# AbrahamSanders/realtime-codec-agent

Hardware: AMD Instinct MI355X
Metric: batch-encode audio-hours/hour (+ xRT and p50 frame-step latency of 1 duplex stream in `duplex`) (higher is better)
Workload: dtype f32; 1 GPU; batch MagiCodec-style encode, 16 kHz stereo, 0.1 s chunks / 2.0 s context, 256 windows per step (BASELINE configs[1]); codebook=131072x16

## Files before the change

include/rca.h:

```cpp
#ifndef RCA_H
#define RCA_H

#include <stdint.h>

#ifdef __cplusplus
extern "C" {
#endif

#define RCA_OK 0
#define RCA_ERR_ARG -1
#define RCA_ERR_HIP -2
#define RCA_ERR_STATE -3
#define RCA_ERR_MISSING -4

#define RCA_MAX_STAGES 8

typedef struct rca_codec rca_codec_t;
typedef struct rca_lm rca_lm_t;

#define RCA_F32 0
#define RCA_BF16 1
#define RCA_Q8_0 2
#define RCA_F16 3
#define RCA_Q6_K 5
// ... 57 lines not shown
typedef struct {
    int64_t src_off;
    int64_t n_in;
    int64_t dst_off;
    int32_t src_stride;
    int32_t n_mix;
} rca_ingest_row_t;
int rca_codec_ingest_rows_dev(rca_codec_t* h, const void* src_dev, int64_t src_span, int32_t src_fmt, const rca_ingest_row_t* rows_dev,
                              const rca_ingest_row_t* rows_host, int32_t n_rows, int32_t up, int32_t down, const float* taps_host,
                              int32_t n_taps, float* dst_dev, int64_t dst_span, void* stream);
int rca_codec_ingest_supported(const rca_codec_t* h, int32_t up, int32_t down, int32_t n_taps);

int rca_codec_encode_tail_dev(rca_codec_t* h, const float* pcm_dev, int32_t B, int32_t T, int32_t n_keep,
                              int64_t* codes_dev, void* stream);
int rca_codec_decode_tail_dev(rca_codec_t* h, const int64_t* codes_dev, int32_t B, int32_t F, int32_t n_samples,
                              float* pcm_dev, void* stream);
int rca_codec_decode_rows_dev(rca_codec_t* h, const int64_t* codes_dev, const int64_t* src_off_dev, int32_t B, int32_t F, int32_t n_samples,
                              float* pcm_dev, const int64_t* dst_off_dev, int64_t code_span, int64_t pcm_span, void* stream);
int rca_codec_decode_error(rca_codec_t* h, void* stream, int32_t* raised);

#define RCA_JOIN_HEAD 1
#define RCA_JOIN_TAIL 2
typedef struct {
    int64_t seg_off;
    int64_t n;
    int64_t out_off;
    int32_t flags;
    int32_t reserved;
} rca_join_seg_t;
int rca_codec_crossfade_join_dev(rca_codec_t* h, const float* seg_dev, int64_t seg_span, const rca_join_seg_t* segs_dev,
                                 const rca_join_seg_t* segs_host, int32_t n_segs, const float* fade_in_dev, int32_t n_fade, float* out_dev,
                                 int64_t out_span, void* stream);

int rca_codec_encode_tail(rca_codec_t* h, const float* pcm_host, int32_t B, int32_t T, int32_t n_keep, int64_t* codes_host);
int rca_codec_decode_tail(rca_codec_t* h, const int64_t* codes_host, int32_t B, int32_t F, int32_t n_samples, float* pcm_host);
int rca_codec_set_stream_graphs(rca_codec_t* h, int32_t enable);
int rca_codec_set_mfma_mode(rca_codec_t* h, int32_t mode);
int rca_codec_receptive_field(const rca_codec_t* h, int32_t* enc_left_frames, int32_t* dec_left_frames);
int rca_codec_set_window_trim(rca_codec_t* h, int32_t enable);

int rca_codec_decode(rca_codec_t* h, const int64_t* codes_host, int32_t B, int32_t F, float* pcm_host);
int rca_codec_decode_dev(rca_codec_t* h, const int64_t* codes_dev, int32_t B, int32_t F, float* pcm_dev,
                         void* stream);

int rca_codec_encoder_dev(rca_codec_t* h, const float* pcm_dev, int32_t B, int32_t T, float* ze_dev, void* stream);
int rca_codec_quantize_dev(rca_codec_t* h, const float* ze_dev, int64_t rows, int64_t* codes_dev, void* stream);
int rca_codec_decoder_dev(rca_codec_t* h, const float* zq_dev, int32_t B, int32_t F, float* pcm_dev, void* stream);
int rca_codec_codebook_dev(rca_codec_t* h, const float** out_dev);

int rca_codec_codebook(rca_codec_t* h, float* out_host);

int rca_codec_encode_tap(rca_codec_t* h, const float* pcm_host, int32_t B, int32_t T, int32_t layer,
                         float* out_host, int64_t out_numel);

int rca_codec_encode_tap_bf16(rca_codec_t* h, const float* pcm_host, int32_t B, int32_t T, int32_t layer,
                              uint16_t* hi_host, uint16_t* lo_host, int64_t numel);

#define RCA_KCLASS_CHAIN 1
#define RCA_KCLASS_MFMA_32x32 2
#define RCA_KCLASS_MFMA_64x32 3
#define RCA_KCLASS_MFMA_32x64 4
#define RCA_KCLASS_MFMA_64x64 5
#define RCA_KCLASS_WS 6
#define RCA_KCLASS_BF16 7
#define RCA_KCLASS_MFMA_OTHER 8
#define RCA_KCLASS_LDS 16
int rca_codec_decoder_layer_tap(rca_codec_t* h, int32_t layer, int32_t route, const float* x_host, int32_t B, int32_t Lin,
                                float* y_host, int64_t y_numel, int32_t* kernel_class, int32_t* guards_ok);

int rca_codec_set_variant(rca_codec_t* h, int32_t variant);

int rca_codec_profile(rca_codec_t* h, int32_t enable);
int rca_codec_profile_read(rca_codec_t* h, int32_t kclass, double* total_ms, int64_t* launches, double* flops,
                           double* bytes);

typedef struct {
    int32_t vocab_size;
    int32_t hidden;
    int32_t n_layers;
    int32_t n_heads;
    int32_t n_kv_heads;
    int32_t head_dim;
    int32_t ffn;
    int32_t n_ctx;
    float rms_eps;
    float rope_theta;
    int32_t rope_scaling;
    float rope_factor;
    float rope_low_freq_factor;
    float rope_high_freq_factor;
    int32_t rope_orig_ctx;
    int32_t logits_all;
    int32_t decode_weights;
} rca_lm_config_t;

typedef struct {
    int32_t top_k;
    float top_p;
    float min_p;
    float temp;
    uint32_t seed;
    int32_t n_bias;
    const int32_t* bias_ids;
    const float* bias_vals;
    float repeat_penalty;
    float freq_penalty;
// ... 135 lines not shown
```

realtime_codec_agent_amd/_native.py:

```python
from __future__ import annotations

import ctypes as C
import os
import subprocess
from typing import Dict, Iterable, List, Optional, Tuple

import numpy as np

_PKG_DIR = os.path.dirname(os.path.abspath(__file__))
CSRC_DIR = os.path.join(_PKG_DIR, "csrc")
LIB_PATH = os.environ.get("RCA_LIB_PATH") or os.path.join(_PKG_DIR, "librca_hip.so")
HIP_SOURCES = ["rca_codec.hip", "rca_lm.hip"]
HIPCC_FLAGS = ["--offload-arch=gfx950", "-O3", "-ffp-contract=off", "-std=c++17", "-fPIC", "-shared",
               "-Wno-unused-result", "-mllvm", "-amdgpu-kernarg-preload-count=14"]

MAX_STAGES = 8
RCA_F32, RCA_BF16, RCA_Q8_0, RCA_F16, RCA_Q4_K, RCA_Q6_K, RCA_Q5_K, RCA_Q4_0, RCA_Q4_1, RCA_IQ4_NL, RCA_IQ4_XS = 0, 1, 2, 3, 4, 5, 6, 7, 8, 9, 10


class RcaError(RuntimeError):
    pass


class Q8Blocks:
# ... 355 lines not shown
    import fcntl
    obj_dir = os.path.join(CSRC_DIR, ".obj")
    os.makedirs(obj_dir, exist_ok=True)
    with open(os.path.join(obj_dir, ".lock"), "w") as lock:
        fcntl.flock(lock, fcntl.LOCK_EX)
        if not force and not needs_build():
            return LIB_PATH
        headers = [os.path.join(CSRC_DIR, f) for f in os.listdir(CSRC_DIR) if f.endswith(".h")]
        headers.append(os.path.join(os.path.dirname(_PKG_DIR), "include", "rca.h"))
        hdr_t = max([os.path.getmtime(p) for p in headers if os.path.exists(p)] + [0.0])
        sfx = f".{os.getpid()}.tmp"
        objs, jobs = [], []
        for src in sources():
            obj = os.path.join(obj_dir, f"{os.path.splitext(os.path.basename(src))[0]}.{key}.o")
            objs.append(obj)
            if force or not os.path.exists(obj) or os.path.getmtime(obj) < max(os.path.getmtime(src), hdr_t):
                cmd = [hipcc] + cflags + ["-c", src, "-o", obj + sfx]
                if verbose:
                    print(" ".join(cmd))
                jobs.append((subprocess.Popen(cmd), cmd, obj))
        tmps = [obj + sfx for _, _, obj in jobs] + [LIB_PATH + sfx]
        try:
            failed = [cmd for p, cmd, _ in jobs if p.wait() != 0]
            if failed:
                raise subprocess.CalledProcessError(1, failed[0])
            for _, _, obj in jobs:
                os.replace(obj + sfx, obj)
            cmd = [hipcc, "--offload-arch=gfx950", "-shared", "-fPIC"] + objs + ["-o", LIB_PATH + sfx]
            if verbose:
                print(" ".join(cmd))
            subprocess.check_call(cmd)
            os.replace(LIB_PATH + sfx, LIB_PATH)
            with open(_stamp_path() + sfx, "w") as f:
                f.write(key + "\n")
            os.replace(_stamp_path() + sfx, _stamp_path())
        finally:
            for t in tmps + [_stamp_path() + sfx]:
                if os.path.exists(t):
                    os.remove(t)
    return LIB_PATH


_lib = None

ABI_SYMBOLS = [
    "rca_last_error", "rca_device_count", "rca_device_sync", "rca_version",
    "rca_codec_create", "rca_codec_destroy", "rca_codec_hop", "rca_codec_num_frames",
    "rca_codec_encode", "rca_codec_encode_dev", "rca_codec_encode_windows_dev", "rca_codec_encode_chunk_range_dev", "rca_codec_encode_rows_dev",
    "rca_codec_ingest_rows_dev", "rca_codec_ingest_supported",
    "rca_codec_decode_rows_dev", "rca_codec_decode_error", "rca_codec_crossfade_join_dev",
    "rca_codec_decode", "rca_codec_decode_dev",
    "rca_codec_encode_tail_dev", "rca_codec_decode_tail_dev", "rca_codec_encode_tail", "rca_codec_decode_tail", "rca_codec_set_stream_graphs", "rca_codec_receptive_field", "rca_codec_set_window_trim",
    "rca_codec_encoder_dev", "rca_codec_quantize_dev", "rca_codec_decoder_dev", "rca_codec_codebook_dev",
    "rca_codec_codebook", "rca_codec_encode_tap", "rca_codec_encode_tap_bf16", "rca_codec_set_variant", "rca_codec_sync",
    "rca_codec_profile", "rca_codec_profile_read",
    "rca_lm_create", "rca_lm_create_random", "rca_lm_destroy", "rca_lm_reset", "rca_lm_eval",
    "rca_lm_get_n_tokens", "rca_lm_set_n_tokens", "rca_lm_get_logits", "rca_lm_get_logits_row",
    "rca_lm_logits_dev", "rca_lm_sampler_init", "rca_lm_sample", "rca_lm_step", "rca_lm_token_probs",
    "rca_lm_sync", "rca_lm_set_graphs", "rca_lm_mask_head_rows", "rca_lm_set_mfma_prefill", "rca_lm_set_logits_all",
    "rca_lm_persist_codec_embeddings", "rca_lm_create_shared", "rca_lm_eval_async", "rca_lm_copy_kv", "rca_lm_swap_kv",
    "rca_lm_set_low_priority", "rca_lm_frame", "rca_lm_weight_format", "rca_lm_set_attn_fuse", "rca_lm_prefill_route",
    "rca_lm_set_act_format", "rca_lm_get_act_format", "rca_lm_gemv_tap", "rca_lm_kv_remove", "rca_lm_kv_read",
    "rca_lm_kv_write", "rca_lm_attn_tap", "rca_lm_score", "rca_lm_score_rows_tap", "rca_lm_put_logits",
    "rca_lm_set_kv_format", "rca_lm_get_kv_format", "rca_lm_kv_bytes_per_position", "rca_lm_kv_read_q8",
    "rca_duplex_frame", "rca_codec_workspace_sig", "rca_codec_stream_handoff", "rca_codec_codebook_size", "rca_codec_set_mfma_mode", "rca_lm_step_probe", "rca_duplex_prepare", "rca_duplex_precapture",
    "rca_lm_group_create", "rca_lm_group_destroy", "rca_lm_group_step",
    "rca_lm_batch_create", "rca_lm_batch_destroy", "rca_lm_batch_step", "rca_lm_batch_frame",
    "rca_lm_batch_frame_sel", "rca_lm_batch_captures", "rca_duplex_batch_frame", "rca_lm_batch_step_sel",
    "rca_lm_batch_eval", "rca_lm_kv_remove_many", "rca_lm_kv_remove_many_staged",
    "rca_codec_decoder_layer_tap", "rca_quantize_rows",
]


def lib():
    global _lib
    if _lib is not None:
        return _lib
    if not os.path.exists(LIB_PATH):
        raise RcaError(
            f"{LIB_PATH} not found: build the HIP extension first (python -c 'import __graft_entry__ as g; g.build()'). "
            "There is no CPU fallback for the product path."
        )
    import torch
    try:
        _lib = C.CDLL(LIB_PATH)
    except OSError as e:
        raise RcaError(f"cannot load {LIB_PATH}: {e}") from e
    _lib.rca_last_error.restype = C.c_char_p
    _lib.rca_version.restype = C.c_char_p
    _lib.rca_lm_batch_step_sel.argtypes = BATCH_STEP_SEL_ARGTYPES
    _lib.rca_lm_batch_step_sel.restype = C.c_int
    if hasattr(_lib, "rca_lm_batch_eval"):
        _lib.rca_lm_batch_eval.argtypes = BATCH_EVAL_ARGTYPES
        _lib.rca_lm_batch_eval.restype = C.c_int
    if hasattr(_lib, "rca_codec_decoder_layer_tap"):
        _lib.rca_codec_decoder_layer_tap.argtypes = DECODER_LAYER_TAP_ARGTYPES
        _lib.rca_codec_decoder_layer_tap.restype = C.c_int
    if hasattr(_lib, "rca_quantize_rows"):
        _lib.rca_quantize_rows.argtypes = QUANTIZE_ROWS_ARGTYPES
        _lib.rca_quantize_rows.restype = C.c_int
    for name in ("rca_lm_kv_remove_many", "rca_lm_kv_remove_many_staged"):
        if hasattr(_lib, name):
            getattr(_lib, name).argtypes = KV_REMOVE_MANY_ARGTYPES
            getattr(_lib, name).restype = C.c_int
    return _lib


# ... 44 lines not shown
```

realtime_codec_agent_amd/codec.py:

```python
from __future__ import annotations

import ctypes as C
from typing import Dict, Optional, Tuple

import numpy as np

from . import _native as N
from .codec_model import CodecConfig, init_codec_weights


class HipCodec:
    def __init__(self, cfg: CodecConfig, weights: Dict[str, np.ndarray], device: int = 0):
        self.cfg = cfg
        self.device = device
        self._lib = N.lib()
        self._h = C.c_void_p()
        tensors, keep = N.make_tensors(weights)
        ccfg = N.codec_config_c(cfg)
        N.check(self._lib.rca_codec_create(C.byref(ccfg), tensors, len(weights), device, C.byref(self._h)), "rca_codec_create")
        del keep
        self.hop = cfg.hop
        self.mfma_mode = 0

    def close(self):
# ... 37 lines not shown
    def encode_tail(self, pcm: np.ndarray, n_keep: int) -> np.ndarray:
        pcm = np.ascontiguousarray(pcm, dtype=np.float32)
        if pcm.ndim != 2:
            raise ValueError("pcm must be [B,T]")
        B, T = pcm.shape
        n_keep = min(int(n_keep), self.num_frames(T))
        codes = np.empty((B, n_keep), np.int64)
        N.check(self._lib.rca_codec_encode_tail(self._h, C.c_void_p(pcm.ctypes.data), B, T, n_keep, C.c_void_p(codes.ctypes.data)),
                "rca_codec_encode_tail")
        return codes

    def decode_tail(self, codes: np.ndarray, n_samples: int) -> np.ndarray:
        codes = np.ascontiguousarray(codes, dtype=np.int64)
        if codes.ndim != 2:
            raise ValueError("codes must be [B,F]")
        B, F = codes.shape
        n = min(int(n_samples), F * self.hop)
        pcm = np.empty((B, n), np.float32)
        N.check(self._lib.rca_codec_decode_tail(self._h, C.c_void_p(codes.ctypes.data), B, F, n, C.c_void_p(pcm.ctypes.data)),
                "rca_codec_decode_tail")
        return pcm

    def set_mfma_mode(self, mode: int) -> None:
        N.check(self._lib.rca_codec_set_mfma_mode(self._h, int(mode)), "rca_codec_set_mfma_mode")
        self.mfma_mode = int(mode)

    def set_stream_graphs(self, enable: bool) -> None:
        N.check(self._lib.rca_codec_set_stream_graphs(self._h, int(bool(enable))), "rca_codec_set_stream_graphs")

    def codebook(self) -> np.ndarray:
        out = np.empty((self.cfg.codebook_size, self.cfg.codebook_dim), np.float32)
        N.check(self._lib.rca_codec_codebook(self._h, C.c_void_p(out.ctypes.data)), "rca_codec_codebook")
        return out

    def encode_tap(self, pcm: np.ndarray, layer: int) -> np.ndarray:
        pcm = np.ascontiguousarray(pcm, dtype=np.float32)
        B, T = pcm.shape
        F = self.num_frames(T)
        n = self.cfg.n_stages
        L = F * self.hop
        if layer == 0:
            shape = (B, self.cfg.channels[0], L)
        elif layer <= n:
            for i in range(layer):
                L //= self.cfg.strides[i]
            shape = (B, self.cfg.channels[layer], L)
        elif layer == n + 1:
            shape = (B, self.cfg.latent_dim, F)
        else:
            shape = (B * F, self.cfg.codebook_dim)
        out = np.empty(shape, np.float32)
        N.check(self._lib.rca_codec_encode_tap(self._h, C.c_void_p(pcm.ctypes.data), B, T, layer, C.c_void_p(out.ctypes.data),
                                               C.c_int64(out.size)), "rca_codec_encode_tap")
        return out

    def encode_tap_bf16(self, pcm: np.ndarray, layer: int) -> Tuple[np.ndarray, Optional[np.ndarray]]:
        pcm = np.ascontiguousarray(pcm, dtype=np.float32)
        B, T = pcm.shape
        L = self.num_frames(T) * self.hop
        for i in range(layer):
            L //= self.cfg.strides[i]
        Cn = self.cfg.channels[layer] if 0 <= layer <= self.cfg.n_stages else 0
        hi = np.empty((B, Cn // 16, L, 16), np.uint16)
        lo = np.empty_like(hi) if self.mfma_mode == 3 else None
        N.check(self._lib.rca_codec_encode_tap_bf16(self._h, C.c_void_p(pcm.ctypes.data), B, T, layer, C.c_void_p(hi.ctypes.data),
                                                    C.c_void_p(lo.ctypes.data if lo is not None else None), C.c_int64(B * Cn * L)),
                "rca_codec_encode_tap_bf16")
        unblock = lambda a: np.ascontiguousarray(a.transpose(0, 1, 3, 2).reshape(B, Cn, L))
        return unblock(hi), (unblock(lo) if lo is not None else None)

    def decoder_layer_tap(self, layer: int, route: int, x: np.ndarray) -> Tuple[np.ndarray, int, bool]:
        x = np.ascontiguousarray(x, dtype=np.float32)
        layers = self.cfg.decoder_layers()
        if x.ndim != 3 or not 0 <= layer < len(layers) or x.shape[1] != layers[layer]["cin"]:
            raise ValueError("x must be [B, Cin, Lin] of a decoder layer")
        ly = layers[layer]
        B, _, Lin = x.shape
        y = np.empty((B, ly["cout"], Lin * ly["s"] if ly["tr"] else Lin), np.float32)
        kclass, guards = C.c_int32(-1), C.c_int32(-1)
        fp = C.POINTER(C.c_float)
        N.check(self._lib.rca_codec_decoder_layer_tap(self._h, layer, route, x.ctypes.data_as(fp), B, Lin, y.ctypes.data_as(fp),
                                                      C.c_int64(y.size), C.byref(kclass), C.byref(guards)), "rca_codec_decoder_layer_tap")
        return y, kclass.value, bool(guards.value)

    def encode_dev(self, pcm_ptr: int, B: int, T: int, codes_ptr: int, stream: int = 0) -> None:
        N.check(self._lib.rca_codec_encode_dev(self._h, C.c_void_p(pcm_ptr), B, T, C.c_void_p(codes_ptr), C.c_void_p(stream)), "rca_codec_encode_dev")

    def decode_dev(self, codes_ptr: int, B: int, F: int, pcm_ptr: int, stream: int = 0) -> None:
        N.check(self._lib.rca_codec_decode_dev(self._h, C.c_void_p(codes_ptr), B, F, C.c_void_p(pcm_ptr), C.c_void_p(stream)), "rca_codec_decode_dev")

    def encode_tail_dev(self, pcm_ptr: int, B: int, T: int, n_keep: int, codes_ptr: int, stream: int = 0) -> None:
        N.check(self._lib.rca_codec_encode_tail_dev(self._h, C.c_void_p(pcm_ptr), B, T, n_keep, C.c_void_p(codes_ptr), C.c_void_p(stream)),
                "rca_codec_encode_tail_dev")

    def decode_tail_dev(self, codes_ptr: int, B: int, F: int, n_samples: int, pcm_ptr: int, stream: int = 0) -> None:
        N.check(self._lib.rca_codec_decode_tail_dev(self._h, C.c_void_p(codes_ptr), B, F, n_samples, C.c_void_p(pcm_ptr), C.c_void_p(stream)),
                "rca_codec_decode_tail_dev")

    def receptive_field(self) -> Tuple[int, int]:
        a, b = C.c_int32(), C.c_int32()
        N.check(self._lib.rca_codec_receptive_field(self._h, C.byref(a), C.byref(b)), "rca_codec_receptive_field")
        return a.value, b.value

    def set_window_trim(self, enable: bool) -> None:
        N.check(self._lib.rca_codec_set_window_trim(self._h, int(bool(enable))), "rca_codec_set_window_trim")

# ... 280 lines not shown
```

realtime_codec_agent_amd/csrc/rca_codec.hip:

```cpp
#include <stdarg.h>

#include <algorithm>
#include <array>
#include <cmath>
#include <map>
#include <type_traits>

#include "rca_common.h"
#include "rca_conv_balance.h"

namespace rca {
thread_local char g_err[512] = {0};
}
using namespace rca;

typedef float f32x16 __attribute__((ext_vector_type(16)));

#define RCA_LAT_MAX_FRAMES 64
#define RCA_LDS_BUDGET (152 * 1024)

typedef float f32x4 __attribute__((ext_vector_type(4)));

struct RowSrc {
    const float* base;
// ... 1508 lines not shown
    for (int ft = 0; ft < FN; ++ft) {
        const long f = f0 + ft * 32 + (lane & 31);
#pragma unroll
        for (int kp = 0; kp < 8; ++kp) zb[ft][kp] = f < F ? z[f * 16 + 2 * kp + half] : 0.0f;
    }
    float best[FN];
    unsigned bidx[FN];
#pragma unroll
    for (int ft = 0; ft < FN; ++ft) { best[ft] = -INFINITY; bidx[ft] = 0xFFFFFFFFu; }

    for (int tile = tile_beg + wave; tile < tile_end; tile += 4) {
        const float4* ap = reinterpret_cast<const float4*>(cbp) + ((long)tile * 2) * 64 + lane;
        const float4 a0 = ap[0], a1 = ap[64];
        const float av[8] = {a0.x, a0.y, a0.z, a0.w, a1.x, a1.y, a1.z, a1.w};
        const int c0 = tile * 32;
        f32x16 cinit;
#pragma unroll
        for (int g = 0; g < 4; ++g) {
            const float4 h4 = *reinterpret_cast<const float4*>(hc + c0 + 8 * g + 4 * half);
            cinit[4 * g + 0] = h4.x; cinit[4 * g + 1] = h4.y; cinit[4 * g + 2] = h4.z; cinit[4 * g + 3] = h4.w;
        }
#pragma unroll
        for (int ft = 0; ft < FN; ++ft) {
            f32x16 acc = cinit;
#pragma unroll
            for (int kp = 0; kp < 8; ++kp) acc = __builtin_amdgcn_mfma_f32_32x32x2f32(av[kp], zb[ft][kp], acc, 0, 0, 0);
#pragma unroll
            for (int r = 0; r < 16; ++r) {
                const unsigned c = (unsigned)(c0 + (r & 3) + 8 * (r >> 2) + 4 * half);
                if (acc[r] > best[ft]) { best[ft] = acc[r]; bidx[ft] = c; }
            }
        }
    }
    __shared__ unsigned long long red[FN][4][32];
#pragma unroll
    for (int ft = 0; ft < FN; ++ft) {
        unsigned long long key = bidx[ft] == 0xFFFFFFFFu ? 0ull : pack_key(best[ft], bidx[ft]);
        const unsigned long long other = __shfl_xor(key, 32);
        key = other > key ? other : key;
        if (lane < 32) red[ft][wave][lane] = key;
    }
    __syncthreads();
    for (int i = threadIdx.x; i < FN * 32; i += 256) {
        const int ft = i >> 5, l = i & 31;
        const long f = f0 + i;
        if (f < F) {
            unsigned long long key = red[ft][0][l];
            for (int w = 1; w < 4; ++w) key = red[ft][w][l] > key ? red[ft][w][l] : key;
            atomicMax(&keys[f], key);
        }
    }
}

struct RowDst {
    int64_t* base;
    int C;
    long chan_stride;
    long win_stride;
    int fc;
    const long* row_off = nullptr;
};
__global__ __launch_bounds__(256) void vq_finalize_kernel(unsigned long long* __restrict__ keys, RowDst dst, long rows) {
    const long i = (long)blockIdx.x * blockDim.x + threadIdx.x;
    if (i >= rows) return;
    const unsigned long long key = keys[i];
    keys[i] = 0ull;
    const long b = i / dst.fc;
    const int j = (int)(i - b * dst.fc);
    dst.base[(dst.row_off ? dst.row_off[b] : (b % dst.C) * dst.chan_stride + (b / dst.C) * dst.win_stride) + j] =
        key == 0ull ? (int64_t)0 : (int64_t)(0xFFFFFFFFu - (unsigned)(key & 0xFFFFFFFFull));
}

__global__ __launch_bounds__(256) void embed_codes_kernel(const int64_t* __restrict__ codes, long ldc, const float* __restrict__ cb,
                                                          float* __restrict__ zq, int B, int F, int J, int N,
                                                          int* __restrict__ err) {
    const long idx = (long)blockIdx.x * blockDim.x + threadIdx.x;
    if (idx >= (long)B * J * F) return;
    const int f = (int)(idx % F);
    const long r = idx / F;
    const int j = (int)(r % J);
    const int b = (int)(r / J);
    int64_t c = codes[(long)b * ldc + f];
    if (c < 0 || c >= N) { atomicExch(err, 1); c = 0; }
    zq[idx] = cb[c * J + j];
}

__global__ __launch_bounds__(256) void embed_rows_kernel(const int64_t* __restrict__ codes, const long* __restrict__ src_off, int f0, int Frow,
                                                         long span, const float* __restrict__ cb, float* __restrict__ zq, int B, int F, int J,
                                                         int N, int* __restrict__ err) {
    const long idx = (long)blockIdx.x * blockDim.x + threadIdx.x;
    if (idx >= (long)B * J * F) return;
    const int f = (int)(idx % F);
    const long r = idx / F;
    const int j = (int)(r % J);
    const int b = (int)(r / J);
    const long o = src_off[b];
    int64_t c = -1;
    if (o >= 0 && o <= span - Frow) c = codes[o + f0 + f];
    if (c < 0 || c >= N) { atomicExch(err, 1); c = 0; }
    zq[idx] = cb[c * J + j];
}

__global__ __launch_bounds__(256) void scatter_tail_kernel(const float* __restrict__ src, long T, int n, float* __restrict__ dst,
                                                           const long* __restrict__ dst_off, long span, int B, int* __restrict__ err) {
    const long idx = (long)blockIdx.x * blockDim.x + threadIdx.x;
    if (idx >= (long)B * n) return;
// ... 1215 lines not shown
        const float slope = c.leaky_slope;
        const int Lout = L / E1.s;
        {
            ProfScope ps(h, st, 0, 2.0 * E1.cin * E1.k * E1.cout * (double)B * Lout + 2.0 * E0.k * E0.cout * (double)B * L,
                         4.0 * ((double)B * src.T + (double)B * E1.cout * Lout + (double)E1.cin * E1.k * E1.cout));
            prev_post = handoff(2, Lout);
            const int act = (E1.pre ? 1 : 0) | (prev_post ? 2 : 0);
            if (h->variant == 2 && try_conv_ws(E1, nullptr, y, B, L, Lout, slope, st, &fin)) { rc = RCA_OK; RCA_LAUNCH_CHECK(); }
            else if (E1.k == 4) rc = launch_conv_mfma<4, 2, 4>(E1, nullptr, y, B, L, Lout, slope, st, &fin, act, h->mfma_mode);
            else if (E1.k == 8) rc = launch_conv_mfma<8, 4, RCA_CIC_K8>(E1, nullptr, y, B, L, Lout, slope, st, &fin, act, h->mfma_mode);
            else rc = launch_conv_mfma<16, 8, RCA_CIC_K16>(E1, nullptr, y, B, L, Lout, slope, st, &fin, act, h->mfma_mode);
        }
        if (rc != RCA_OK) return rc;
        L = Lout;
        first = 2;
        if (tap_layer == 1) RCA_HIP(hipMemcpyAsync(tap_dev, y, (size_t)B * E1.cout * L * 4, hipMemcpyDeviceToDevice, st));
    } else if (h->lat_mode && !src.row_off && src.win_stride == 0 && src.C == B &&
               try_conv_lds(h, h->enc[0], src.base, src.chan_stride, src.T, h->act[cur].as<float>(), B, L, 0, st)) {
        RCA_LAUNCH_CHECK();
    } else {
        const ConvLayer& L0 = h->enc[0];
        const long total = (long)B * L;
        float* y = h->act[cur].as<float>();
        ProfScope ps(h, st, 2, 2.0 * L0.k * L0.cout * (double)total, 4.0 * ((double)total + (double)total * L0.cout));
        if (L0.k == 7) conv_in_kernel<7><<<cdiv(total, 256), 256, 0, st>>>(src, L0.w, L0.b, y, B, L0.cout, L);
        else if (L0.k == 5) conv_in_kernel<5><<<cdiv(total, 256), 256, 0, st>>>(src, L0.w, L0.b, y, B, L0.cout, L);
        else conv_in_kernel<3><<<cdiv(total, 256), 256, 0, st>>>(src, L0.w, L0.b, y, B, L0.cout, L);
        RCA_LAUNCH_CHECK();
        if (tap_layer == 0) RCA_HIP(hipMemcpyAsync(tap_dev, y, (size_t)B * L0.cout * L * 4, hipMemcpyDeviceToDevice, st));
    }
    for (size_t li = first; li < h->enc.size(); ++li) {
        const ConvLayer& Ly = h->enc[li];
        float* x = h->act[cur].as<float>();
        float* y = h->act[cur ^ 1].as<float>();
        bool done = false;
        int view = 0;
        if (li + 1 == h->enc.size() && Fz_out && keep > 0 && tap_layer < 0 && !Ly.tr) {
            const char* hk = getenv("RCA_HEAD_KEEP");
            const int want = keep + conv_view_halo(Ly);
            if (!(hk && hk[0] == '0') && want < L / Ly.s && conv_view_ok(h, Ly, B, L, want)) view = want;
        }
        if ((rc = run_conv(h, Ly, x, y, B, L, 0, st, prev_post, handoff(li + 1, L / Ly.s), &done, view)) != RCA_OK) return rc;
        if (view) *Fz_out = view;
        prev_post = done;
        L /= Ly.s;
        cur ^= 1;
        if (tap_layer == (int)li) RCA_HIP(hipMemcpyAsync(tap_dev, y, (size_t)B * Ly.cout * L * 4, hipMemcpyDeviceToDevice, st));
    }
    *ze_out = h->act[cur].as<float>();
    *F_out = F;
    return RCA_OK;
}

static int run_quantize(rca_codec* h, const float* ze, int ze_is_rows, int B, int F, int f0, int fc, RowDst dst, hipStream_t st,
                        float* ztap_dev) {
    const rca_codec_config_t& c = h->cfg;
    const long rows = (long)B * fc;
    const int J = c.codebook_dim, N = c.codebook_size;
    int rc;
    if ((rc = h->zbuf.ensure((size_t)rows * J * 4)) != RCA_OK) return rc;
    const size_t need_keys = (size_t)rows;
    if (h->keys.cap < need_keys * 8) {
        if ((rc = h->keys.ensure(need_keys * 8)) != RCA_OK) return rc;
        RCA_HIP(hipMemsetAsync(h->keys.p, 0, h->keys.cap, st));
    }
    float* z = h->zbuf.as<float>();
    in_proj_kernel<<<cdiv(rows * J, 256), 256, 0, st>>>(ze, h->q_in_w, h->q_in_b, z, B, c.latent_dim, F, f0, fc, J, ze_is_rows);
    RCA_LAUNCH_CHECK();
    if (ztap_dev) RCA_HIP(hipMemcpyAsync(ztap_dev, z, (size_t)rows * J * 4, hipMemcpyDeviceToDevice, st));
    unsigned long long* keys = h->keys.as<unsigned long long>();
    ProfScope ps(h, st, 1, 2.0 * (double)rows * N * J, 4.0 * ((double)N * (J + 1) + (double)rows * J) + 8.0 * rows);
    if (h->variant >= 1) {
        constexpr int FN = 2;
        const int ftiles = (int)cdiv(rows, FN * 32);
        const int total_tiles = N / 32;
        int splits = (int)std::max(1L, std::min((long)total_tiles / 16, (1024 + ftiles - 1) / (long)ftiles));
        int tps = (total_tiles + splits - 1) / splits;
        tps = (tps + 3) / 4 * 4;
        splits = (total_tiles + tps - 1) / tps;
        dim3 grid(ftiles, splits);
        vq_mfma_kernel<FN><<<grid, 256, 0, st>>>(z, h->cbp, h->hc, keys, rows, N, tps);
    } else {
        constexpr int FB = 4;
        const int fblocks = (int)cdiv(rows, FB);
        int splits = (int)std::max(1L, std::min((long)N / 1024, (1024 + fblocks - 1) / (long)fblocks));
        int cps = (N + splits - 1) / splits;
        cps = (cps + 255) / 256 * 256;
        splits = (N + cps - 1) / cps;
        dim3 grid(fblocks, splits);
        vq_chain_kernel<FB><<<grid, 256, 0, st>>>(z, h->cb, h->hc, keys, rows, N, cps);
    }
    RCA_LAUNCH_CHECK();
    dst.fc = fc;
    vq_finalize_kernel<<<cdiv(rows, 256), 256, 0, st>>>(keys, dst, rows);
    RCA_LAUNCH_CHECK();
    return RCA_OK;
}

static hipStream_t pick_stream(rca_codec* h, void* stream) {
    hipStream_t st = (hipStream_t)stream;
    if (h->last_stream_valid && h->last_stream != st) {
        if (!h->xev) (void)hipEventCreateWithFlags(&h->xev, hipEventDisableTiming);
        (void)hipEventRecord(h->xev, h->last_stream);
        (void)hipStreamWaitEvent(st, h->xev, 0);
    }
    h->last_stream = st;
    h->last_stream_valid = true;
    return st;
}

extern "C" int rca_codec_encode_dev(rca_codec_t* h, const float* pcm, int32_t B, int32_t T, int64_t* codes, void* stream) {
    if (!h || !pcm || !codes || B < 1 || T < 1) return fail(RCA_ERR_ARG, "encode: bad argument (B=%d T=%d)", B, T);
    RCA_HIP(hipSetDevice(h->device));
    hipStream_t st = pick_stream(h, stream);
    RowSrc src{pcm, B, (long)T, 0, T};
    float* ze; int F, rc;
    if ((rc = run_encoder(h, src, B, st, &ze, &F, -1, nullptr)) != RCA_OK) return rc;
    RowDst dst{codes, B, (long)F, 0, F};
    return run_quantize(h, ze, 0, B, F, 0, F, dst, st, nullptr);
}

static int trimmable_frames(const rca_codec* h, int F, int keep) { return std::max(0, F - keep - h->enc_left_frames); }

extern "C" int rca_codec_encode_tail_dev(rca_codec_t* h, const float* pcm, int32_t B, int32_t T, int32_t n_keep, int64_t* codes,
                                         void* stream) {
// ... 123 lines not shown
        return fail(RCA_ERR_ARG, "codes buffer too small: %ld < %ld", (long)codes_per_channel, (long)(chunk_end - chunk_begin) * fpc);
    const int W = std::max(chunk, ctx);
    int rc;
    long i = chunk_begin;
    for (; i < chunk_end && (i + 1) * (long)chunk < W; ++i) {
        const int Tfull = (int)((i + 1) * chunk);
        const int jw = h->window_trim ? trimmable_frames(h, (Tfull + h->hop - 1) / h->hop, fpc) : 0;
        const int T = Tfull - jw * h->hop;
        RowSrc src{audio + (long)jw * h->hop, C, (long)N, 0, T};
        float* ze; int F, Fz;
        if ((rc = run_encoder(h, src, C, st, &ze, &F, -1, nullptr, -1, nullptr, fpc, &Fz)) != RCA_OK) return rc;
        if (F < fpc) return fail(RCA_ERR_STATE, "window of %d samples has %d frames < %d kept", T, F, fpc);
        RowDst dst{codes + (i - chunk_begin) * fpc, C, (long)codes_per_channel, 0, fpc};
        if ((rc = run_quantize(h, ze, 0, C, Fz, Fz - fpc, fpc, dst, st, nullptr)) != RCA_OK) return rc;
    }
    const int wins_per_pass = std::max(1, batch_windows / C);
    while (i < chunk_end) {
        const int nw = (int)std::min<long>(wins_per_pass, chunk_end - i);
        const int jw = h->window_trim ? trimmable_frames(h, (W + h->hop - 1) / h->hop, fpc) : 0;
        const long start0 = (i + 1) * (long)chunk - W + (long)jw * h->hop;
        RowSrc src{audio + start0, C, (long)N, (long)chunk, W - jw * h->hop};
        float* ze; int F, Fz;
        if ((rc = run_encoder(h, src, nw * C, st, &ze, &F, -1, nullptr, -1, nullptr, fpc, &Fz)) != RCA_OK) return rc;
        if (F < fpc) return fail(RCA_ERR_STATE, "window has %d frames < %d kept", F, fpc);
        RowDst dst{codes + (i - chunk_begin) * fpc, C, (long)codes_per_channel, (long)fpc, fpc};
        if ((rc = run_quantize(h, ze, 0, nw * C, Fz, Fz - fpc, fpc, dst, st, nullptr)) != RCA_OK) return rc;
        i += nw;
    }
    return RCA_OK;
}

extern "C" int rca_codec_encode_windows_dev(rca_codec_t* h, const float* audio, int32_t C, int64_t N, int32_t chunk, int32_t ctx,
                                            int32_t batch_windows, int64_t* codes, int64_t codes_per_channel, void* stream) {
    if (chunk < 1) return fail(RCA_ERR_ARG, "encode_windows: bad argument");
    return rca_codec_encode_chunk_range_dev(h, audio, C, N, chunk, ctx, batch_windows, 0, N / chunk, codes, codes_per_channel, stream);
}

extern "C" int rca_codec_encode_rows_dev(rca_codec_t* h, const float* audio, const int64_t* src_off, int32_t B, int32_t T, int32_t n_keep,
                                         int64_t* codes, const int64_t* dst_off, int64_t span, void* stream) {
    if (!h || !audio || !src_off || !codes || !dst_off || B < 1 || T < 1 || n_keep < 1 || span < T)
        return fail(RCA_ERR_ARG, "encode_rows: bad argument");
    RCA_HIP(hipSetDevice(h->device));
    hipStream_t st = pick_stream(h, stream);
    static_assert(sizeof(long) == sizeof(int64_t), "offset tables are 64-bit");
    const int Ffull = (T + h->hop - 1) / h->hop;
    if (Ffull < n_keep) return fail(RCA_ERR_ARG, "encode_rows: a window of %d samples has %d frames < %d kept", T, Ffull, n_keep);
    const int jw = h->window_trim ? trimmable_frames(h, Ffull, n_keep) : 0;
    RowSrc src{audio + (long)jw * h->hop, B, 0, 0, T - jw * h->hop, reinterpret_cast<const long*>(src_off), (long)span};
    float* ze; int F, Fz;
    int rc;
    if ((rc = run_encoder(h, src, B, st, &ze, &F, -1, nullptr, -1, nullptr, n_keep, &Fz)) != RCA_OK) return rc;
    RowDst dst{codes, B, 0, 0, n_keep, reinterpret_cast<const long*>(dst_off)};
    return run_quantize(h, ze, 0, B, Fz, Fz - n_keep, n_keep, dst, st, nullptr);
}

#define RCA_INGEST_TILE 256
#define RCA_INGEST_SPAN (8 * RCA_INGEST_TILE)
#define RCA_INGEST_LDS_BUDGET (64 * 1024)

__device__ __forceinline__ float ingest_cvt(float v) { return v; }
__device__ __forceinline__ float ingest_cvt(int16_t v) { return (float)v * 0x1p-15f; }

template <typename S>
__device__ __forceinline__ float ingest_frame(const S* __restrict__ src, long off, int n_mix) {
    float a = ingest_cvt(src[off]);
    if (n_mix > 1) {
        for (int c = 1; c < n_mix; ++c) a += ingest_cvt(src[off + c]);
        a = a / (float)n_mix;
    }
    return a;
}

template <typename S>
__global__ __launch_bounds__(RCA_INGEST_TILE) void ingest_rows_kernel(const S* __restrict__ src, const rca_ingest_row_t* __restrict__ rows,
                                                                      int up, int down, int half, int jmax, int pitch,
                                                                      const float* __restrict__ ph_tab, float* __restrict__ dst) {
    extern __shared__ float ingest_lds[];
    float* ph = ingest_lds;
    float* xs = ingest_lds + (long)up * pitch;
    const rca_ingest_row_t r = rows[blockIdx.y];
    const long n_out = (r.n_in * up + down - 1) / down;
    long n0 = (long)blockIdx.x * RCA_INGEST_SPAN;
    if (n0 >= n_out) return;
    const long n_end = n0 + RCA_INGEST_SPAN < n_out ? n0 + RCA_INGEST_SPAN : n_out;
    const int tid = threadIdx.x;
    if (up == 1 && down == 1) {
        for (long n = n0 + tid; n < n_end; n += RCA_INGEST_TILE) dst[r.dst_off + n] = ingest_frame(src, r.src_off + n * r.src_stride, r.n_mix);
        return;
    }
    for (int i = tid; i < up * pitch; i += RCA_INGEST_TILE) ph[i] = ph_tab[i];
    for (; n0 < n_end; n0 += RCA_INGEST_TILE) {
        const int cnt = (int)(n_end - n0 < RCA_INGEST_TILE ? n_end - n0 : RCA_INGEST_TILE);
        const long k_first = (n0 * down + half) / up - (jmax - 1);
        const long k_last = ((n0 + cnt - 1) * down + half) / up;
        const int span = (int)(k_last - k_first + 1);
        __syncthreads();
        for (int i = tid; i < span; i += RCA_INGEST_TILE) {
            const long k = k_first + i;
            xs[i] = (k >= 0 && k < r.n_in) ? ingest_frame(src, r.src_off + k * r.src_stride, r.n_mix) : 0.0f;
        }
        __syncthreads();
        if (tid < cnt) {
            const long t = (n0 + tid) * down + half;
            const long kh = t / up;
            const float* pr = ph + (t - kh * up) * pitch;
            const float* xr = xs + (kh - k_first);
// ... 493 lines not shown
```

Before: 3483 audio-hours/hour.

## Add fast VQ argmax kernel with prefetch and occupancy-based split geometry

Adds a double-buffered MFMA nearest-code search kernel that prefetches the next codebook tile, reduces the per-row max with v_max3 and a ballot-guarded index update, and sizes the codebook split count from the device's CU count and kernel occupancy. Also adds an LDS-tiled in-projection kernel for the frame-major latent layout, and a host tap entry point for checking the kept-frame latents and projected rows. The aim is to cut time spent in the 131072-entry codebook search and the in-projection on the batch-encode path. Both paths are enabled by default through an environment switch and fall back when the geometry check fails.

```diff
diff --git a/include/rca.h b/include/rca.h
--- a/include/rca.h
+++ b/include/rca.h
@@ -133,6 +133,9 @@
 
 int rca_codec_encode_tap(rca_codec_t* h, const float* pcm_host, int32_t B, int32_t T, int32_t layer,
                          float* out_host, int64_t out_numel);
+
+int rca_codec_encode_keep_tap(rca_codec_t* h, const float* pcm_host, int32_t B, int32_t T, int32_t n_keep, int32_t what,
+                              float* out_host, int64_t out_numel);
 
 int rca_codec_encode_tap_bf16(rca_codec_t* h, const float* pcm_host, int32_t B, int32_t T, int32_t layer,
                               uint16_t* hi_host, uint16_t* lo_host, int64_t numel);
diff --git a/realtime_codec_agent_amd/_native.py b/realtime_codec_agent_amd/_native.py
--- a/realtime_codec_agent_amd/_native.py
+++ b/realtime_codec_agent_amd/_native.py
@@ -431,7 +431,7 @@
     "rca_codec_decode", "rca_codec_decode_dev",
     "rca_codec_encode_tail_dev", "rca_codec_decode_tail_dev", "rca_codec_encode_tail", "rca_codec_decode_tail", "rca_codec_set_stream_graphs", "rca_codec_receptive_field", "rca_codec_set_window_trim",
     "rca_codec_encoder_dev", "rca_codec_quantize_dev", "rca_codec_decoder_dev", "rca_codec_codebook_dev",
-    "rca_codec_codebook", "rca_codec_encode_tap", "rca_codec_encode_tap_bf16", "rca_codec_set_variant", "rca_codec_sync",
+    "rca_codec_codebook", "rca_codec_encode_tap", "rca_codec_encode_keep_tap", "rca_codec_encode_tap_bf16", "rca_codec_set_variant", "rca_codec_sync",
     "rca_codec_profile", "rca_codec_profile_read",
     "rca_lm_create", "rca_lm_create_random", "rca_lm_destroy", "rca_lm_reset", "rca_lm_eval",
     "rca_lm_get_n_tokens", "rca_lm_set_n_tokens", "rca_lm_get_logits", "rca_lm_get_logits_row",
diff --git a/realtime_codec_agent_amd/codec.py b/realtime_codec_agent_amd/codec.py
--- a/realtime_codec_agent_amd/codec.py
+++ b/realtime_codec_agent_amd/codec.py
@@ -113,6 +113,15 @@
         out = np.empty(shape, np.float32)
         N.check(self._lib.rca_codec_encode_tap(self._h, C.c_void_p(pcm.ctypes.data), B, T, layer, C.c_void_p(out.ctypes.data),
                                                C.c_int64(out.size)), "rca_codec_encode_tap")
+        return out
+
+    def encode_keep_tap(self, pcm: np.ndarray, n_keep: int, what: int) -> np.ndarray:
+        pcm = np.ascontiguousarray(pcm, dtype=np.float32)
+        B, T = pcm.shape
+        shape = (B, self.cfg.latent_dim, n_keep) if what == 0 else (B * n_keep, self.cfg.codebook_dim)
+        out = np.empty(shape, np.float32)
+        N.check(self._lib.rca_codec_encode_keep_tap(self._h, C.c_void_p(pcm.ctypes.data), B, T, int(n_keep), int(what),
+                                                    C.c_void_p(out.ctypes.data), C.c_int64(out.size)), "rca_codec_encode_keep_tap")
         return out
 
     def encode_tap_bf16(self, pcm: np.ndarray, layer: int) -> Tuple[np.ndarray, Optional[np.ndarray]]:
diff --git a/realtime_codec_agent_amd/csrc/rca_codec.hip b/realtime_codec_agent_amd/csrc/rca_codec.hip
--- a/realtime_codec_agent_amd/csrc/rca_codec.hip
+++ b/realtime_codec_agent_amd/csrc/rca_codec.hip
@@ -1584,6 +1584,148 @@
     }
 }
 
+struct VqFrag { float4 a0, a1, h0, h1, h2, h3; };
+__device__ __forceinline__ void vq_load_frag(VqFrag& f, const float* __restrict__ cbp, const float* __restrict__ hc, int tile, int lane) {
+    const float4* ap = reinterpret_cast<const float4*>(cbp) + ((long)tile * 2) * 64 + lane;
+    const float4* hp = reinterpret_cast<const float4*>(hc + (long)tile * 32 + 4 * (lane >> 5));
+    f.a0 = ap[0]; f.a1 = ap[64];
+    f.h0 = hp[0]; f.h1 = hp[2]; f.h2 = hp[4]; f.h3 = hp[6];
+}
+__device__ __forceinline__ float vq_max3(float a, float b, float c) {
+    float m;
+    asm("v_max3_f32 %0, %1, %2, %3" : "=v"(m) : "v"(a), "v"(b), "v"(c));
+    return m;
+}
+template <int FN>
+__device__ __forceinline__ void vq_tile(const VqFrag& f, const float (&zb)[FN][8], float (&best)[FN], unsigned (&bsel)[FN], int tile) {
+    const float av[8] = {f.a0.x, f.a0.y, f.a0.z, f.a0.w, f.a1.x, f.a1.y, f.a1.z, f.a1.w};
+    const f32x16 cinit = {f.h0.x, f.h0.y, f.h0.z, f.h0.w, f.h1.x, f.h1.y, f.h1.z, f.h1.w,
+                          f.h2.x, f.h2.y, f.h2.z, f.h2.w, f.h3.x, f.h3.y, f.h3.z, f.h3.w};
+#pragma unroll
+    for (int ft = 0; ft < FN; ++ft) {
+        f32x16 acc = cinit;
+#pragma unroll
+        for (int kp = 0; kp < 8; ++kp) acc = __builtin_amdgcn_mfma_f32_32x32x2f32(av[kp], zb[ft][kp], acc, 0, 0, 0);
+        float m = vq_max3(acc[0], acc[1], acc[2]);
+#pragma unroll
+        for (int r = 3; r < 15; r += 2) m = vq_max3(m, acc[r], acc[r + 1]);
+        m = vq_max3(m, acc[15], acc[15]);
+        if (__builtin_amdgcn_ballot_w64(m > best[ft]) != 0ull) {
+            const float before = best[ft];
+            unsigned rsel = 0;
+#pragma unroll
+            for (int r = 0; r < 16; ++r)
+                if (acc[r] > best[ft]) { best[ft] = acc[r]; rsel = (unsigned)r; }
+            if (best[ft] > before) bsel[ft] = (unsigned)tile * 32u + rsel;
+        }
+    }
+}
+template <int FN>
+__global__ __launch_bounds__(256) void vq_mfma_fast_kernel(const float* __restrict__ z, const float* __restrict__ cbp,
+                                                           const float* __restrict__ hc, unsigned long long* __restrict__ keys,
+                                                           long F, int N, int tiles_per_split) {
+    const int lane = threadIdx.x & 63;
+    const int wave = __builtin_amdgcn_readfirstlane(threadIdx.x >> 6);
+    const int split = blockIdx.y;
+    const long f0 = (long)blockIdx.x * (FN * 32);
+    const int last_tile = N / 32 - 1;
+    const int tile_beg = split * tiles_per_split;
+    const int tile_end = min(N / 32, tile_beg + tiles_per_split);
+    const int half = lane >> 5;
+
+    int tile = tile_beg + wave;
+    VqFrag fa, fb;
+    vq_load_frag(fa, cbp, hc, min(tile, last_tile), lane);
+    float zb[FN][8];
+#pragma unroll
+    for (int ft = 0; ft < FN; ++ft) {
+        const long f = f0 + ft * 32 + (lane & 31);
+#pragma unroll
+        for (int kp = 0; kp < 8; ++kp) zb[ft][kp] = z[min(f, F - 1) * 16 + 2 * kp + half];
+    }
+    float best[FN];
+    unsigned bsel[FN];
+#pragma unroll
+    for (int ft = 0; ft < FN; ++ft) { best[ft] = -INFINITY; bsel[ft] = 0xFFFFFFFFu; }
+
+    while (tile < tile_end) {
+        vq_load_frag(fb, cbp, hc, min(tile + 4, last_tile), lane);
+        vq_tile<FN>(fa, zb, best, bsel, tile);
+        tile += 4;
+        if (tile >= tile_end) break;
+        vq_load_frag(fa, cbp, hc, min(tile + 4, last_tile), lane);
+        vq_tile<FN>(fb, zb, best, bsel, tile);
+        tile += 4;
+    }
+    __shared__ unsigned long long red[FN][4][32];
+#pragma unroll
+    for (int ft = 0; ft < FN; ++ft) {
+        const unsigned r = bsel[ft] & 31u;
+        const unsigned c = (bsel[ft] & ~31u) + (r & 3u) + 8u * (r >> 2) + 4u * (unsigned)half;
+        unsigned long long key = bsel[ft] == 0xFFFFFFFFu ? 0ull : pack_key(best[ft], c);
+        const unsigned long long other = __shfl_xor(key, 32);
+        key = other > key ? other : key;
+        if (lane < 32) red[ft][wave][lane] = key;
+    }
+    __syncthreads();
+    for (int i = threadIdx.x; i < FN * 32; i += 256) {
+        const int ft = i >> 5, l = i & 31;
+        const long f = f0 + i;
+        if (f < F) {
+            unsigned long long key = red[ft][0][l];
+            for (int w = 1; w < 4; ++w) key = red[ft][w][l] > key ? red[ft][w][l] : key;
+            atomicMax(&keys[f], key);
+        }
+    }
+}
+
+constexpr int RCA_INPROJ_RT = 16, RCA_INPROJ_DC = 256;
+__global__ __launch_bounds__(256) void in_proj_rows_kernel(const float* __restrict__ ze, const float* __restrict__ w,
+                                                           const float* __restrict__ bias, float* __restrict__ z, long rows,
+                                                           int D, int F, int f0, int fc, int J) {
+    constexpr int RT = RCA_INPROJ_RT, DC = RCA_INPROJ_DC;
+    constexpr int P = DC + 4;
+    __shared__ __attribute__((aligned(16))) float xs[RT * P];
+    __shared__ __attribute__((aligned(16))) float ws[16 * P];
+    const long r0 = (long)blockIdx.x * RT;
+    const int tid = threadIdx.x;
+    const int rr = tid / J, j = tid - rr * J;
+    const bool mine = rr < RT && r0 + rr < rows;
+    float acc = mine ? bias[j] : 0.0f;
+    const long rs = min(r0 + (tid & (RT - 1)), rows - 1);
+    const long bs = rs / fc;
+    const float* zsrc = ze + bs * D * F + (f0 + (int)(rs - bs * fc));
+    for (int d0 = 0; d0 < D; d0 += DC) {
+        const int dc = min(DC, D - d0);
+        float xv[DC / 16], wv[16];
+#pragma unroll
+        for (int k = 0; k < DC / 16; ++k) xv[k] = zsrc[(long)min(d0 + (tid >> 4) + 16 * k, D - 1) * F];
+#pragma unroll
+        for (int k = 0; k < 16; ++k) wv[k] = w[(long)min(k, J - 1) * D + min(d0 + tid, D - 1)];
+        if (d0) __syncthreads();
+#pragma unroll
+        for (int k = 0; k < DC / 16; ++k) xs[(tid & (RT - 1)) * P + (tid >> 4) + 16 * k] = xv[k];
+#pragma unroll
+        for (int k = 0; k < 16; ++k) ws[k * P + tid] = wv[k];
+        __syncthreads();
+        if (mine) {
+            const float* xp = xs + rr * P;
+            const float* wp = ws + j * P;
+            int d = 0;
+#pragma unroll 4
+            for (; d + 4 <= dc; d += 4) {
+                const float4 x4 = *reinterpret_cast<const float4*>(xp + d), w4 = *reinterpret_cast<const float4*>(wp + d);
+                acc = __builtin_fmaf(w4.x, x4.x, acc);
+                acc = __builtin_fmaf(w4.y, x4.y, acc);
+                acc = __builtin_fmaf(w4.z, x4.z, acc);
+                acc = __builtin_fmaf(w4.w, x4.w, acc);
+            }
+            for (; d < dc; ++d) acc = __builtin_fmaf(wp[d], xp[d], acc);
+        }
+    }
+    if (mine) z[(r0 + rr) * J + j] = acc;
+}
+
 struct RowDst {
     int64_t* base;
     int C;
@@ -2905,6 +3047,36 @@
     return RCA_OK;
 }
 
+static bool head_fast() {
+    const char* hf = getenv("RCA_HEAD_FAST");
+    return !(hf && hf[0] == '0');
+}
+
+struct VqGeom { int splits, tps; };
+static bool vq_geometry(long rows, int total_tiles, VqGeom* out) {
+    if (rows < 1 || total_tiles < 1) return false;
+    const long ftiles = cdiv(rows, 64);
+    if (ftiles >= (1L << 31) || total_tiles > 65535 * 16) return false;
+    long splits = 0;
+    if (const char* e = getenv("RCA_VQ_GEOM")) splits = std::min(std::min((long)total_tiles, 65535L), std::max(0L, atol(e)));
+    const bool forced = splits > 0;
+    if (!forced) {
+        static long resident_of[64];
+        int dev = 0;
+        if (hipGetDevice(&dev) != hipSuccess || dev < 0 || dev >= 64) return false;
+        if (!resident_of[dev]) {
+            int cus = 0, blocks = 0;
+            if (hipDeviceGetAttribute(&cus, hipDeviceAttributeMultiprocessorCount, dev) != hipSuccess || cus <= 0) return false;
+            if (hipOccupancyMaxActiveBlocksPerMultiprocessor(&blocks, vq_mfma_fast_kernel<2>, 256, 0) != hipSuccess || blocks < 1) return false;
+            resident_of[dev] = (long)cus * std::min(blocks, 8);
+        }
+        splits = std::max(1L, std::min(std::max(1L, (long)total_tiles / 16), resident_of[dev] / ftiles));
+    }
+    const int tps = (int)cdiv(total_tiles, splits);
+    *out = VqGeom{(int)cdiv(total_tiles, tps), tps};
+    return forced || tps >= 32;
+}
+
 static int run_quantize(rca_codec* h, const float* ze, int ze_is_rows, int B, int F, int f0, int fc, RowDst dst, hipStream_t st,
                         float* ztap_dev) {
     const rca_codec_config_t& c = h->cfg;
@@ -2918,12 +3090,20 @@
         RCA_HIP(hipMemsetAsync(h->keys.p, 0, h->keys.cap, st));
     }
     float* z = h->zbuf.as<float>();
-    in_proj_kernel<<<cdiv(rows * J, 256), 256, 0, st>>>(ze, h->q_in_w, h->q_in_b, z, B, c.latent_dim, F, f0, fc, J, ze_is_rows);
+    const bool fast = head_fast() && h->variant >= 1;
+    if (fast && !ze_is_rows && J <= 16)
+        in_proj_rows_kernel<<<(unsigned)cdiv(rows, RCA_INPROJ_RT), 256, 0, st>>>(ze, h->q_in_w, h->q_in_b, z, rows, c.latent_dim, F, f0, fc, J);
+    else
+        in_proj_kernel<<<cdiv(rows * J, 256), 256, 0, st>>>(ze, h->q_in_w, h->q_in_b, z, B, c.latent_dim, F, f0, fc, J, ze_is_rows);
     RCA_LAUNCH_CHECK();
     if (ztap_dev) RCA_HIP(hipMemcpyAsync(ztap_dev, z, (size_t)rows * J * 4, hipMemcpyDeviceToDevice, st));
     unsigned long long* keys = h->keys.as<unsigned long long>();
     ProfScope ps(h, st, 1, 2.0 * (double)rows * N * J, 4.0 * ((double)N * (J + 1) + (double)rows * J) + 8.0 * rows);
-    if (h->variant >= 1) {
+    VqGeom g;
+    if (fast && vq_geometry(rows, N / 32, &g)) {
+        const dim3 grid((unsigned)cdiv(rows, 64), (unsigned)g.splits);
+        vq_mfma_fast_kernel<2><<<grid, 256, 0, st>>>(z, h->cbp, h->hc, keys, rows, N, g.tps);
+    } else if (h->variant >= 1) {
         constexpr int FN = 2;
         const int ftiles = (int)cdiv(rows, FN * 32);
         const int total_tiles = N / 32;
@@ -3153,6 +3333,49 @@
     if ((rc = run_encoder(h, src, B, st, &ze, &F, -1, nullptr, -1, nullptr, n_keep, &Fz)) != RCA_OK) return rc;
     RowDst dst{codes, B, 0, 0, n_keep, reinterpret_cast<const long*>(dst_off)};
     return run_quantize(h, ze, 0, B, Fz, Fz - n_keep, n_keep, dst, st, nullptr);
+}
+
+extern "C" int rca_codec_encode_keep_tap(rca_codec_t* h, const float* pcm_host, int32_t B, int32_t T, int32_t n_keep, int32_t what,
+                                         float* out_host, int64_t out_numel) {
+    if (!h || !pcm_host || !out_host || B < 1 || T < 1 || n_keep < 1 || (what != 0 && what != 1)) return fail(RCA_ERR_ARG, "keep tap: bad argument");
+    RCA_HIP(hipSetDevice(h->device));
+    const int Ffull = (T + h->hop - 1) / h->hop;
+    if (Ffull < n_keep) return fail(RCA_ERR_ARG, "keep tap: a window of %d samples has %d frames < %d kept", T, Ffull, n_keep);
+    const int D = h->cfg.latent_dim, J = h->cfg.codebook_dim;
+    const long want = what == 0 ? (long)B * D * n_keep : (long)B * n_keep * J;
+    if (want != out_numel) return fail(RCA_ERR_ARG, "keep tap: out_numel %ld, expected %ld", (long)out_numel, want);
+    int rc;
+    if ((rc = h->io_a.ensure((size_t)B * T * 4)) != RCA_OK) return rc;
+    if ((rc = h->io_b.ensure((size_t)out_numel * 4)) != RCA_OK) return rc;
+    std::vector<int64_t> off((size_t)2 * B);
+    for (int b = 0; b < B; ++b) { off[b] = (int64_t)b * T; off[B + b] = (int64_t)b * n_keep; }
+    DevBuf tmp;
+    if ((rc = tmp.ensure(((size_t)2 * B + (size_t)B * n_keep) * 8)) != RCA_OK) return rc;
+    hipStream_t st = pick_stream(h, h->stream);
+    auto run = [&]() -> int {
+        RCA_HIP(hipMemcpyAsync(h->io_a.p, pcm_host, (size_t)B * T * 4, hipMemcpyHostToDevice, st));
+        RCA_HIP(hipMemcpyAsync(tmp.p, off.data(), (size_t)2 * B * 8, hipMemcpyHostToDevice, st));
+        const long* offs = tmp.as<long>();
+        const int jw = h->window_trim ? trimmable_frames(h, Ffull, n_keep) : 0;
+        RowSrc src{h->io_a.as<float>() + (long)jw * h->hop, B, 0, 0, T - jw * h->hop, offs, (long)B * T};
+        float* ze; int F, Fz, r;
+        if ((r = run_encoder(h, src, B, st, &ze, &F, -1, nullptr, -1, nullptr, n_keep, &Fz)) != RCA_OK) return r;
+        if (what == 0) {
+            RCA_HIP(hipMemcpy2DAsync(h->io_b.p, (size_t)n_keep * 4, ze + (Fz - n_keep), (size_t)Fz * 4, (size_t)n_keep * 4, (size_t)B * D,
+                                     hipMemcpyDeviceToDevice, st));
+        } else {
+            RowDst dst{tmp.as<int64_t>() + 2 * B, B, 0, 0, n_keep, offs + B};
+            if ((r = run_quantize(h, ze, 0, B, Fz, Fz - n_keep, n_keep, dst, st, h->io_b.as<float>())) != RCA_OK) return r;
+        }
+        RCA_HIP(hipMemcpyAsync(out_host, h->io_b.p, (size_t)out_numel * 4, hipMemcpyDeviceToHost, st));
+        return RCA_OK;
+    };
+    rc = run();
+    const hipError_t e = hipStreamSynchronize(st);
+    tmp.release();
+    if (rc != RCA_OK) return rc;
+    if (e != hipSuccess) return fail(RCA_ERR_HIP, "keep tap sync: %s", hipGetErrorString(e));
+    return RCA_OK;
 }
 
 #define RCA_INGEST_TILE 256
```

Result: no change. 3514 audio-hours/hour, median of 6 (+0.9%).
